# usnistgov/optbayesexpt

Hardware: AMD Instinct MI355X
Metric: model-evals/sec (settings x particles) per opt_setting+update cycle, fp64 (higher is better)
Workload: dtype f64; 1 GPU; c3: Lorentzian 3-param, 65 536 settings x 1 048 576 particles; n_settings=65536, n_particles=1048576, settings_per_rank=65536

## Files before the change

### optbayesexpt_amd/csrc/obe_sweep_bins.h

```cpp
#pragma once
#include "obe_sweep_common.h"

namespace obe {

struct BinPlan {
    double origin;
    int nbins;
    unsigned poison;
};
constexpr int kBinMinmaxBlocks = 256;
constexpr int kBinMaxUnits = 2048;
constexpr int kBinChunk = 1024;
constexpr int kBinFoldGroups = 16;
constexpr int kBinScanPer = kBinMaxUnits / kBlock;
constexpr double kBinEvalSlots = 8.0 * LorentzBins::kOrder + 16.0;
constexpr double kBinDrawSlots = 4.0 * LorentzBins::kOrder + 8.0;
constexpr double kBinFixedSlots = 80.0 * 3.9e7;

struct BinUnits {
    int nunits;
    int64_t per;
};
static BinUnits plan_bin_units(int64_t nd) {
    BinUnits u;
    u.per = (nd + kBinMaxUnits - 1) / kBinMaxUnits;
    u.per = std::max<int64_t>(kWave, (u.per + kWave - 1) / kWave * kWave);
    u.nunits = static_cast<int>((nd + u.per - 1) / u.per);
    return u;
}
struct BinEvalShape {
    int waves, groups;
};
constexpr BinEvalShape kBinEvalShapes[] = {{8, 1}, {6, 2}, {3, 4}};
constexpr int kBinEvalWavesPerCU = 12, kChipCUs = 256;
static int plan_bin_eval_waves(int64_t ns) {
    const int64_t groups = (ns + kWave - 1) / kWave;
    for (const BinEvalShape& f : kBinEvalShapes)
        if (groups <= (int64_t)kChipCUs * f.groups * (kBinEvalWavesPerCU / (f.groups * f.waves))) return f.waves;
    return 1;
}
static int64_t bin_max_items(int64_t nd) { return (nd + kBinChunk - 1) / kBinChunk + LorentzBins::kMaxBins; }
struct BinLayout {
    static constexpr int64_t kPlan = 0, kRan = 3, kStarts = 4;
    static constexpr int64_t kMinmax = kStarts + 132;
    static constexpr int64_t kTotals = kMinmax + 3 * kBinMinmaxBlocks;
    static constexpr int64_t kCounts = kTotals + LorentzBins::kMaxBins / 2;
    static constexpr int64_t kCoef = kCounts + (int64_t)LorentzBins::kMaxBins * kBinMaxUnits / 2;
    static constexpr int64_t kPart = kCoef + (int64_t)LorentzBins::kMaxBins * LorentzBins::kRow;
    static int64_t sorted(int64_t nd) { return kPart + bin_max_items(nd) * LorentzBins::kRow; }
    static int64_t doubles(int64_t nd) { return sorted(nd) + 4 * nd; }
};
static_assert(BinLayout::kPart % 2 == 0 && LorentzBins::kRow % 2 == 0, "the sorted records are 16-byte aligned");

struct BinKeep {
    BinPlan plan;
    unsigned mark;
    int nd;
    unsigned long long dbits;
    unsigned mismatch;
    unsigned records;
    unsigned pad[6];
};
static_assert(sizeof(BinKeep) == 64, "the head of the keep buffer is 16 ints");
constexpr unsigned kBinKeepMark = 0x6b455042u;
struct BinKeepLayout {
    static constexpr int64_t kStarts = sizeof(BinKeep) / sizeof(int);
    static constexpr int64_t kDest = (kStarts + 2 * (LorentzBins::kMaxBins + 2) + 3) & ~(int64_t)3;
    static int64_t bytes(int64_t nd) { return ((kDest + nd) * (int64_t)sizeof(int) + 15) & ~(int64_t)15; }
    static constexpr int64_t kRecord = 3;
    static int64_t records_at(int64_t nd) { return bytes(nd); }
    static int64_t sw_at(int64_t nd) { return records_at(nd) + ((kRecord * 8 * nd + 15) & ~(int64_t)15); }
    static int64_t records_bytes(int64_t nd) { return sw_at(nd) + ((8 * nd + 15) & ~(int64_t)15); }
};

#ifndef OBE_PLUGIN_MODEL_HEADER
struct BinSweepPtrs {
    BinPlan* plan;
    unsigned* ran;
    int* binstart;
    int* itemstart;
    BinKeep* keep;
    int* dest;
    int* code;
    int reuse;
    int keep_nd;
    unsigned long long keep_dbits;
    unsigned call;
    double* minmax;
    int* totals;
    int* counts;
    double* coef;
    double* part;
    double* sorted;
};

struct BinRecords {
    double* rec;
    double* sw;
    const double* bbar;
};

__device__ __forceinline__ bool bin_keep_refused(const BinSweepPtrs& q) {
    if (!q.reuse) return false;
    const BinKeep* k = q.keep;
    return !(k->mark == kBinKeepMark && k->nd == q.keep_nd && k->dbits == q.keep_dbits);
}

__device__ __forceinline__ double bin_x0(const SweepArgs& a, int64_t p) {
    double w;
    const int64_t src = draw_source(a, p, w);
    return a.particles[src];
}
__device__ __forceinline__ double bin_tau0(const SweepArgs& a, int64_t p) { return bin_x0(a, p) / a.m.consts[0]; }

__device__ __forceinline__ void bin_pk(double tau0, double amp, double b, double bbar, double sw, double (&pk)[4]) {
    pk[0] = tau0;
    pk[1] = sw * amp;
    pk[2] = sw * (b - bbar);
    pk[3] = sw;
}
__device__ __forceinline__ void bin_particle(const SweepArgs& a, int64_t p, double (&part)[3], double& sw) {
    using M = Lorentz<1>;
    static_assert(packed_width<M>() == 4 && M::NPK == 3, "the sorted records are 32 bytes");
    double w;
    const int64_t src = draw_source(a, p, w);
    sw = sqrt(w);
    part[0] = a.particles[src] / a.m.consts[0];
    part[1] = a.particles[src + a.ld_p];
    part[2] = a.particles[src + 2 * a.ld_p];
}
__device__ __forceinline__ void bin_record(const SweepArgs& a, int64_t p, double2& ra, double2& rb) {
    double part[3], sw, pk[4];
    bin_particle(a, p, part, sw);
    bin_pk(part[0], part[1], part[2], a.moments[4], sw, pk);
    ra = double2{pk[0], pk[1]};
    rb = double2{pk[2], pk[3]};
}

__device__ __forceinline__ void bin_store_particle(const SweepArgs& a, int64_t p, int pos, const BinRecords& r) {
    double part[3], sw;
    bin_particle(a, p, part, sw);
    double* __restrict__ out = r.rec + BinKeepLayout::kRecord * (int64_t)pos;
    out[0] = part[0];
    out[1] = part[1];
    out[2] = part[2];
    r.sw[pos] = sw;
}

constexpr int kBinRankBits = 24;
static_assert((((int64_t)1 << 30) + kBinMaxUnits - 1) / kBinMaxUnits <= ((int64_t)1 << kBinRankBits)
                  && LorentzBins::kMaxBins <= (1 << (31 - kBinRankBits)),
              "a unit of a cloud of 2^30 draws (BinForm::selected) has at most 2^19 draws: rank and bin share an int");
__device__ __forceinline__ int bin_code(int bin, int rank) { return (bin << kBinRankBits) | rank; }
constexpr int kBinIndexBits = 7;
constexpr int kBinGroupAhead = 8;
static_assert(LorentzBins::kMaxBins == 1 << kBinIndexBits, "a bin index is matched bit by bit (bin_group_kernel<false>)");

__global__ __launch_bounds__(kBlock) void bin_minmax_kernel(SweepArgs a, BinSweepPtrs q) {
    constexpr int NW = kBlock / kWave;
    __shared__ double slo[NW], shi[NW];
    __shared__ int sbad[NW];
    if (sweep_aborted(a.abort)) return;
    if (q.keep && blockIdx.x == 0 && threadIdx.x == 0) {
        q.keep->mark = 0u;
        q.keep->records = 0u;
    }
    double* __restrict__ minmax = q.minmax;
    double lo = INFINITY, hi = -INFINITY;
    int bad = 0;
    for (int64_t p = (int64_t)blockIdx.x * kBlock + threadIdx.x; p < a.nd; p += (int64_t)gridDim.x * kBlock) {
        const double t = bin_tau0(a, p);
        bad |= !(fabs(t) <= kDblMax);
        lo = fmin(lo, t);
        hi = fmax(hi, t);
    }
#pragma unroll
    for (int o = kWave / 2; o > 0; o >>= 1) {
        lo = fmin(lo, __shfl_down(lo, o, kWave));
        hi = fmax(hi, __shfl_down(hi, o, kWave));
        bad |= __shfl_down(bad, o, kWave);
    }
    if ((threadIdx.x & (kWave - 1)) == 0) {
        slo[threadIdx.x / kWave] = lo;
        shi[threadIdx.x / kWave] = hi;
        sbad[threadIdx.x / kWave] = bad;
    }
    __syncthreads();
    if (threadIdx.x != 0) return;
    for (int g = 1; g < NW; ++g) {
        lo = fmin(lo, slo[g]);
        hi = fmax(hi, shi[g]);
        bad |= sbad[g];
    }
    minmax[blockIdx.x] = lo;
    minmax[kBinMinmaxBlocks + blockIdx.x] = hi;
    minmax[2 * kBinMinmaxBlocks + blockIdx.x] = bad ? 1.0 : 0.0;
}

__device__ __forceinline__ BinPlan bin_plan_of(const SweepArgs& a, const double* __restrict__ minmax, int nblocks) {
    const int lane = threadIdx.x & (kWave - 1);
    double lo = INFINITY, hi = -INFINITY;
    int bad = 0;
#pragma unroll
    for (int g = 0; g < kBinMinmaxBlocks / kWave; ++g) {
        const int b = g * kWave + lane;
        const bool have = b < nblocks;
        lo = fmin(lo, have ? minmax[b] : INFINITY);
        hi = fmax(hi, have ? minmax[kBinMinmaxBlocks + b] : -INFINITY);
        bad |= have ? minmax[2 * kBinMinmaxBlocks + b] != 0.0 : 0;
    }
#pragma unroll
    for (int o = kWave / 2; o > 0; o >>= 1) {
        lo = fmin(lo, __shfl_xor(lo, o, kWave));
        hi = fmax(hi, __shfl_xor(hi, o, kWave));
        bad |= __shfl_xor(bad, o, kWave);
    }
    const double d = a.m.consts[0];
    const double n = floor((hi - lo) * (1.0 / LorentzBins::kWidth)) + 1.0;
    const bool ok = !bad && d > 0.0 && d <= kDblMax && fabs(lo) <= kDblMax && fabs(hi) <= kDblMax
                    && n <= (double)LorentzBins::kMaxBins;
    return BinPlan{lo, ok ? static_cast<int>(n) : 0, ok ? 0u : 1u};
}

__device__ __forceinline__ int wave_exclusive(int v, int& total) {
    const int lane = threadIdx.x & (kWave - 1);
    int inc = v;
#pragma unroll
    for (int o = 1; o < kWave; o <<= 1) {
        const int up = __shfl_up(inc, o, kWave);
        inc += lane >= o ? up : 0;
    }
    total = __shfl(inc, kWave - 1, kWave);
    return inc - v;
}

template <bool SCATTER, bool RECORDS = false>
__global__ __launch_bounds__(kBlock) void bin_group_kernel(SweepArgs a, int64_t per, int nunits, int mm_blocks,
                                                           BinSweepPtrs q, BinRecords r) {
    using LB = LorentzBins;
    static_assert(SCATTER || !RECORDS, "the counting pass stores no record");
    if (sweep_aborted(a.abort)) return;
    const int lane = threadIdx.x & (kWave - 1);
    const int unit = blockIdx.x * (kBlock / kWave) + threadIdx.x / kWave;
    BinPlan plan;
    if constexpr (SCATTER) {
        plan = *q.plan;
        if (q.keep && blockIdx.x == 0 && threadIdx.x == 0) {
            q.keep->nd = static_cast<int>(a.nd);
            q.keep->dbits = q.keep_dbits;
            q.keep->mismatch = 0u;
            q.keep->mark = kBinKeepMark;
            if constexpr (RECORDS) q.keep->records = kBinKeepMark;
        }
    } else {
        plan = bin_plan_of(a, q.minmax, mm_blocks);
        if (blockIdx.x == 0 && threadIdx.x == 0) *q.plan = plan;
    }
    const int nbins = __builtin_amdgcn_readfirstlane(plan.nbins);
    if (nbins == 0) return;
    int c0 = 0, c1 = 0;
    if constexpr (SCATTER) {
        const int t0 = q.totals[lane], t1 = q.totals[lane + kWave];
        int sum0, sum1, isum0, isum1;
        const int e0 = wave_exclusive(t0, sum0), e1 = sum0 + wave_exclusive(t1, sum1);
        const int i0 = wave_exclusive((t0 + kBinChunk - 1) / kBinChunk, isum0);
        const int i1 = isum0 + wave_exclusive((t1 + kBinChunk - 1) / kBinChunk, isum1);
        if (unit == 0) {
            q.binstart[lane] = e0;
            q.binstart[lane + kWave] = e1;
            q.itemstart[lane] = i0;
            q.itemstart[lane + kWave] = i1;
            if (lane == 0) {
                q.binstart[LB::kMaxBins] = sum0 + sum1;
                q.itemstart[LB::kMaxBins] = isum0 + isum1;
            }
        }
        if (unit >= nunits) return;
        c0 = e0 + q.counts[lane * kBinMaxUnits + unit];
        c1 = e1 + q.counts[(lane + kWave) * kBinMaxUnits + unit];
    }
    if (unit >= nunits) return;
    const int64_t begin = (int64_t)unit * per;
    const int64_t end = begin + per < a.nd ? begin + per : a.nd;
    if constexpr (SCATTER) {
        for (int64_t i0 = begin; i0 < end; i0 += kWave) {
            const int64_t i = i0 + lane;
            const bool live = i < end;
            const int code = live ? q.code[i] : 0;
            const int bin = code >> kBinRankBits;
            const int first0 = __shfl(c0, bin & (kWave - 1), kWave), first1 = __shfl(c1, bin & (kWave - 1), kWave);
            const int pos = (bin < kWave ? first0 : first1) + (code & ((1 << kBinRankBits) - 1));
            if (live && pos >= 0 && pos < a.nd) {
                if constexpr (RECORDS) {
                    bin_store_particle(a, i, pos, r);
                } else {
                    double2 ra, rb;
                    bin_record(a, i, ra, rb);
                    double2* __restrict__ out = reinterpret_cast<double2*>(q.sorted) + 2 * (int64_t)pos;
                    out[0] = ra;
                    out[1] = rb;
                }
            }
            if (q.dest && live) q.dest[i] = pos;
        }
    } else {
        __shared__ int tally[kBlock / kWave][LB::kMaxBins];
        int* count = tally[threadIdx.x / kWave];
        count[lane] = 0;
        count[lane + kWave] = 0;
        __builtin_amdgcn_fence(__ATOMIC_SEQ_CST, "wavefront");
        const double d = a.m.consts[0];
        const unsigned long long below = (1ull << lane) - 1ull;
        auto trip = [&](int64_t i0, double x0) {
            const int64_t i = i0 + lane;
            const bool live = i < end;
            const int bin = live ? LB::bin_of(plan.origin, x0 / d, nbins) : -1;
            unsigned long long same = __ballot(live);
#pragma unroll
            for (int k = 0; k < kBinIndexBits; ++k) {
                const bool bit = (bin >> k) & 1;
                const unsigned long long have = __ballot(bit);
                same &= bit ? have : ~have;
            }
            if (!live) same = 0ull;
            const int sofar = live ? count[bin] : 0;
            if (live && (same & below) == 0ull) count[bin] = sofar + __popcll(same);
            __builtin_amdgcn_fence(__ATOMIC_SEQ_CST, "wavefront");
            if (live) q.code[i] = bin_code(bin, sofar + __popcll(same & below));
        };
        for (int64_t i0 = begin; i0 < end; i0 += kBinGroupAhead * kWave) {
            double x0[kBinGroupAhead];
#pragma unroll
            for (int k = 0; k < kBinGroupAhead; ++k) {
                const int64_t i = i0 + k * kWave + lane;
                x0[k] = bin_x0(a, i < end ? i : end - 1);
            }
#pragma unroll
            for (int k = 0; k < kBinGroupAhead; ++k)
                if (i0 + k * kWave < end) trip(i0 + k * kWave, x0[k]);
        }
        q.counts[lane * kBinMaxUnits + unit] = count[lane];
        q.counts[(lane + kWave) * kBinMaxUnits + unit] = count[lane + kWave];
    }
}

template <bool RECORDS>
__device__ __forceinline__ void bin_scatter_pack_draw(const SweepArgs& a, const BinSweepPtrs& q, const BinRecords& r,
                                                      double origin, int nbins, int64_t p) {
    using LB = LorentzBins;
    double2 ra, rb;
    bin_record(a, p, ra, rb);
    const int pos = q.dest[p];
    const double t = (ra.x - origin) * (1.0 / LB::kWidth);
    bool ok = t >= 0.0 && t < (double)nbins && pos >= 0 && pos < a.nd;
    if (ok) {
        const int b = LB::bin_of(origin, ra.x, nbins);
        ok = q.binstart[b] <= pos && pos < q.binstart[b + 1];
    }
    if (ok) {
        if constexpr (RECORDS) {
            bin_store_particle(a, p, pos, r);
        } else {
            double2* __restrict__ out = reinterpret_cast<double2*>(q.sorted) + 2 * (int64_t)pos;
            out[0] = ra;
            out[1] = rb;
        }
    } else {
        q.keep->mismatch = q.call;
    }
}
__global__ __launch_bounds__(kBlock) void bin_scatter_pack_kernel(SweepArgs a, BinSweepPtrs q) {
    using LB = LorentzBins;
    if (sweep_aborted(a.abort)) return;
    if (bin_keep_refused(q)) return;
    const int nbins = __builtin_amdgcn_readfirstlane(q.plan->nbins);
    if (nbins <= 0 || nbins > LB::kMaxBins) return;
    const double origin = q.plan->origin;
    for (int64_t p = (int64_t)blockIdx.x * kBlock + threadIdx.x; p < a.nd; p += (int64_t)gridDim.x * kBlock)
        bin_scatter_pack_draw<false>(a, q, BinRecords{}, origin, nbins, p);
}

__global__ __launch_bounds__(kBlock) void bin_refresh_kernel(SweepArgs a, BinSweepPtrs q, BinRecords r, int64_t per) {
    using LB = LorentzBins;
    if (sweep_aborted(a.abort)) return;
    if (bin_keep_refused(q)) return;
    const int nbins = __builtin_amdgcn_readfirstlane(q.plan->nbins);
    if (nbins <= 0 || nbins > LB::kMaxBins) return;
    const int64_t begin = (int64_t)blockIdx.x * per;
    const int64_t end = begin + per < a.nd ? begin + per : a.nd;
    if (q.keep->records == kBinKeepMark) {
        const double* __restrict__ w = a.weights;
        const int* __restrict__ dest = q.dest;
        for (int64_t p = begin + threadIdx.x; p < end; p += kBlock) {
            const int pos = dest[p];
            if (pos >= 0 && pos < a.nd) r.sw[pos] = sqrt(w[p]);
        }
    } else {
        const double origin = q.plan->origin;
        for (int64_t p = begin + threadIdx.x; p < end; p += kBlock) bin_scatter_pack_draw<true>(a, q, r, origin, nbins, p);
    }
}

__global__ __launch_bounds__(kBlock) void bin_scan_kernel(int nunits, BinSweepPtrs q, const unsigned* abort) {
    __shared__ int wsum[kBlock / kWave];
    if (sweep_aborted(abort)) return;
    const int nbins = __builtin_amdgcn_readfirstlane(q.plan->nbins);
    const int bin = blockIdx.x;
    if (nbins == 0) return;
    if (bin >= nbins) {
        if (threadIdx.x == 0) q.totals[bin] = 0;
        return;
    }
    int* __restrict__ row = q.counts + bin * kBinMaxUnits;
    int v[kBinScanPer], mine = 0;
#pragma unroll
    for (int u = 0; u < kBinScanPer; ++u) {
        const int k = threadIdx.x * kBinScanPer + u;
        v[u] = k < nunits ? row[k] : 0;
        mine += v[u];
    }
    int wtotal;
    int before = wave_exclusive(mine, wtotal);
    if ((threadIdx.x & (kWave - 1)) == 0) wsum[threadIdx.x / kWave] = wtotal;
    __syncthreads();
    int total = 0;
#pragma unroll
    for (int g = 0; g < kBlock / kWave; ++g) {
        if (g < (int)threadIdx.x / kWave) before += wsum[g];
        total += wsum[g];
    }
#pragma unroll
    for (int u = 0; u < kBinScanPer; ++u) {
        const int k = threadIdx.x * kBinScanPer + u;
        if (k < nunits) row[k] = before;
        before += v[u];
    }
    if (threadIdx.x == 0) q.totals[bin] = total;
}

template <int N, int DIST>
__device__ __forceinline__ void halving_reduce(const double (&v)[N], int lane, double (&out)[2]) {
    constexpr int H = (N + 1) / 2;
    const bool upper = (lane & DIST) != 0;
    double k[H];
#pragma unroll
    for (int i = 0; i < H; ++i) {
        const double lo = v[i], hi = H + i < N ? v[H + i] : 0.0;
        const double mine = upper ? hi : lo, send = upper ? lo : hi;
        k[i] = mine + __shfl_xor(send, DIST, kWave);
    }
    if constexpr (DIST > 1) {
        halving_reduce<H, DIST / 2>(k, lane, out);
    } else {
        static_assert(H == 2, "64 lanes x 2 values: at most 128 sums");
        out[0] = k[0];
        out[1] = k[1];
    }
}
template <int N>
__device__ __forceinline__ int halving_index(int lane, int e) {
    int n[7];
    n[0] = N;
#pragma unroll
    for (int l = 0; l < 6; ++l) n[l + 1] = (n[l] + 1) / 2;
    int j = e;
    bool real = true;
#pragma unroll
    for (int l = 5; l >= 0; --l) {
        j += ((lane >> (5 - l)) & 1) * n[l + 1];
        real = real && j < n[l];
    }
    return real ? j : -1;
}

template <bool RECORDS>
__global__ __launch_bounds__(kWave) void bin_moments_kernel(BinSweepPtrs q, const unsigned* abort, BinRecords r) {
    using LB = LorentzBins;
    if (sweep_aborted(abort)) return;
    if (bin_keep_refused(q)) return;
    const int nbins = __builtin_amdgcn_readfirstlane(q.plan->nbins);
    if (nbins == 0) return;
    const int lane = threadIdx.x, item = blockIdx.x;
    if (item >= q.itemstart[LB::kMaxBins]) return;
    const int s0 = q.itemstart[lane], s1 = q.itemstart[lane + kWave];
    const int bin = __popcll(__ballot(lane < nbins && s0 <= item)) + __popcll(__ballot(lane + kWave < nbins && s1 <= item)) - 1;
    const int first = q.binstart[bin] + (item - q.itemstart[bin]) * kBinChunk;
    const int last = q.binstart[bin + 1];
    const int end = first + kBinChunk < last ? first + kBinChunk : last;
    const double tb = LB::centre(q.plan->origin, bin);
    LB::Sums z;
    z.clear();
    if constexpr (!RECORDS) {
        const double2* __restrict__ rec = reinterpret_cast<const double2*>(q.sorted);
        int i = first + lane;
        double2 ra = double2{0.0, 0.0}, rb = ra;
        if (i < end) {
            ra = rec[2 * (int64_t)i];
            rb = rec[2 * (int64_t)i + 1];
        }
        while (i < end) {
            const int in = i + kWave;
            double2 na = ra, nb = rb;
            if (in < end) {
                na = rec[2 * (int64_t)in];
                nb = rec[2 * (int64_t)in + 1];
            }
            const double pk[4] = {ra.x, ra.y, rb.x, rb.y};
            LB::add_draw(tb, pk, z);
            ra = na;
            rb = nb;
            i = in;
        }
    } else {
        const double bbar = *r.bbar;
        const double* __restrict__ rec = r.rec;
        const double* __restrict__ rsw = r.sw;
        constexpr int64_t R = BinKeepLayout::kRecord;
        int i = first + lane;
        double tau0 = 0.0, amp = 0.0, b = 0.0, sw = 0.0;
        if (i < end) {
            tau0 = rec[R * i];
            amp = rec[R * i + 1];
            b = rec[R * i + 2];
            sw = rsw[i];
        }
        while (i < end) {
            const int in = i + kWave;
            double ntau0 = tau0, namp = amp, nb = b, nsw = sw;
            if (in < end) {
                ntau0 = rec[R * in];
                namp = rec[R * in + 1];
                nb = rec[R * in + 2];
                nsw = rsw[in];
            }
            double pk[4];
            bin_pk(tau0, amp, b, bbar, sw, pk);
            LB::add_draw(tb, pk, z);
            tau0 = ntau0;
            amp = namp;
            b = nb;
            sw = nsw;
            i = in;
        }
    }
    double v[LB::kCoefs], kept[2];
#pragma unroll
    for (int k = 0; k < LB::kOrder; ++k) {
        v[k] = z.M1[k];
        v[LB::kOrder + k] = z.M2[k];
        v[2 * LB::kOrder + k] = z.M3[k];
    }
    v[3 * LB::kOrder] = z.c1;
    v[3 * LB::kOrder + 1] = z.c2;
    halving_reduce<LB::kCoefs, kWave / 2>(v, lane, kept);
    double* __restrict__ out = q.part + (int64_t)item * LB::kRow;
#pragma unroll
    for (int e = 0; e < 2; ++e) {
        const int j = halving_index<LB::kCoefs>(lane, e);
        if (j < 0) continue;
        const bool m3 = j >= 2 * LB::kOrder && j < 3 * LB::kOrder;
        out[j] = kept[e] * (m3 ? (double)(j - 2 * LB::kOrder + 1) : 1.0);
    }
}

__global__ __launch_bounds__(kBinFoldGroups * kWave) void bin_fold_kernel(BinSweepPtrs q, const unsigned* abort) {
    using LB = LorentzBins;
    __shared__ double acc[kBinFoldGroups][kWave];
    if (sweep_aborted(abort)) return;
    if (bin_keep_refused(q)) return;
    const int nbins = __builtin_amdgcn_readfirstlane(q.plan->nbins);
    const int bin = blockIdx.x >> 1, co = (blockIdx.x & 1) * kWave + (threadIdx.x & (kWave - 1));
    if (bin >= nbins) return;
    const int first = __builtin_amdgcn_readfirstlane(q.itemstart[bin]);
    const int n = __builtin_amdgcn_readfirstlane(q.itemstart[bin + 1]) - first;
    if (n == 0) return;
    const bool live = co < LB::kCoefs;
    const double t = fold_in_order<kBinFoldGroups>(q.part + (int64_t)first * LB::kRow + co, n, LB::kRow, live, acc);
    if (threadIdx.x < kWave && live) q.coef[(int64_t)bin * LB::kRow + co] = t;
}

constexpr int kBinTile = 16;
template <int G, int W>
__global__ __launch_bounds__(G * W * kWave, W == 1 ? 1 : 3)
void bin_eval_kernel(SweepArgs a, BinSweepPtrs q, unsigned seq, BinFinish f) {
    using LB = LorentzBins;
    constexpr int kThreads = G * W * kWave;
    static_assert(W > 1 || kThreads == kBlock, "W = 1 is the workgroup of four groups");
    static_assert((G * W) % 4 == 0, "whole wavefronts for every SIMD of the CU (plan_bin_eval_waves)");
    static_assert(LB::kMaxBins <= 2 * kWave && kWave % kBinTile == 0, "two ballots name the occupied bins");
    const int lane = threadIdx.x & (kWave - 1);
    const int wave = __builtin_amdgcn_readfirstlane((int)threadIdx.x / kWave);
    const int grp = wave % G, wid = wave / G;
    double* term = nullptr;
    if constexpr (W == 1) {
        if (sweep_aborted(a.abort)) return;
    } else {
        __shared__ double terms[G * 2 * kBinTile * kWave];
        __shared__ int stop;
        term = terms + grp * (2 * kBinTile * kWave);
        if (threadIdx.x == 0) stop = sweep_aborted(a.abort);
        __syncthreads();
        if (stop) return;
    }
    const int64_t s = ((int64_t)blockIdx.x * G + grp) * kWave + lane;
    const bool refused = bin_keep_refused(q) || (q.reuse && q.keep->mismatch == q.call);
    const int nbins = refused ? 0 : __builtin_amdgcn_readfirstlane(q.plan->nbins);
    double S1 = __builtin_nan(""), S2 = __builtin_nan("");
    if (nbins > 0) {
        double tau;
        Lorentz<1>::prep_setting(a.settings + (s < a.ns ? s : a.ns - 1), a.m, &tau);
        const double origin = q.plan->origin;
        const double* __restrict__ coef = q.coef;
        const int* __restrict__ start = q.binstart;
        const bool here0 = lane < nbins && start[lane + 1] != start[lane];
        const bool here1 = kWave + lane < nbins && start[kWave + lane + 1] != start[kWave + lane];
        const uint64_t occ0 = __ballot(here0), occ1 = __ballot(here1);
        uint64_t own0 = occ0, own1 = occ1;
        double c1col[2] = {0.0, 0.0}, c2col[2] = {0.0, 0.0};
        if constexpr (W > 1) {
            uint64_t mine = 0;
            for (int t = wid; t < kBinTile; t += W) mine |= (uint64_t)1 << t;
            mine |= mine << 16;
            mine |= mine << 32;
            own0 &= mine;
            own1 &= mine;
            if (wid == 0) {
                if (here0) {
                    c1col[0] = coef[lane * LB::kRow + 3 * LB::kOrder];
                    c2col[0] = coef[lane * LB::kRow + 3 * LB::kOrder + 1];
                }
                if (here1) {
                    c1col[1] = coef[(kWave + lane) * LB::kRow + 3 * LB::kOrder];
                    c2col[1] = coef[(kWave + lane) * LB::kRow + 3 * LB::kOrder + 1];
                }
            }
        }
        auto next_bin = [&]() {
            int b = -1;
            if (own0) {
                b = __builtin_ctzll(own0);
                own0 &= own0 - 1;
            } else if (own1) {
                b = kWave + __builtin_ctzll(own1);
                own1 &= own1 - 1;
            }
            return b;
        };
        double a1 = 0.0, a2 = 0.0, C1 = 0.0, C2 = 0.0;
        int tile = 0;
        auto close_tile = [&]() {
            __syncthreads();
            if (wid == 0) {
                const int half = tile * kBinTile / kWave;
                const uint64_t occ = half ? occ1 : occ0;
                for (int t = 0; t < kBinTile; ++t) {
                    const int l = (tile * kBinTile + t) & (kWave - 1);
                    if (!((occ >> l) & 1)) continue;
                    a1 += term[t * kWave + lane];
                    a2 += term[(kBinTile + t) * kWave + lane];
                    C1 += readlane_f64(half ? c1col[1] : c1col[0], l);
                    C2 += readlane_f64(half ? c2col[1] : c2col[0], l);
                }
            }
            __syncthreads();
            ++tile;
        };
        auto evaluate = [&](const LB::LaneRow& row, int b) {
            double t1, t2;
            if constexpr (W == 1) {
                LB::evaluate(row, LB::centre(origin, b) - tau, t1, t2);
                a1 += t1;
                a2 += t2;
                LB::add_constants(row, C1, C2);
            } else {
                while (tile < b / kBinTile) close_tile();
                LB::evaluate(row, LB::centre(origin, b) - tau, t1, t2);
                term[(b % kBinTile) * kWave + lane] = t1;
                term[(kBinTile + b % kBinTile) * kWave + lane] = t2;
            }
        };
        LB::LaneRow row0, row1;
        int b0 = next_bin();
        if (b0 >= 0) {
            LB::load_row(coef + b0 * LB::kRow, lane, row0);
            for (;;) {
                const int b1 = next_bin();
                LB::load_row(coef + (b1 >= 0 ? b1 : b0) * LB::kRow, lane, row1);
                evaluate(row0, b0);
                if (b1 < 0) break;
                b0 = next_bin();
                LB::load_row(coef + (b0 >= 0 ? b0 : b1) * LB::kRow, lane, row0);
                evaluate(row1, b1);
                if (b0 < 0) break;
            }
        }
        if constexpr (W > 1)
            while (tile < (nbins + kBinTile - 1) / kBinTile) close_tile();
        S1 = a1 + C1;
        S2 = a2 + C2;
    }
    if (blockIdx.x == 0 && threadIdx.x == 0) *q.ran = seq;
    if (W > 1 && wid != 0) return;
    if (!f.yvar) {
        if (s >= a.ns) return;
        a.part1[s] = S1;
        a.part2[s] = S2;
        a.cs_out[s] = 0.0;
        return;
    }
    const int64_t group = (int64_t)blockIdx.x * G + grp;
    if (group * kWave >= a.ns) return;
    double kappa = 0.0;
    Best best{-INFINITY, INT64_MAX};
    if (s < a.ns) {
        const double var = variance_of_moments(0.0 + S1, 0.0 + S2, f.full_mode ? a.moments[0] : 1.0, 0.0, kappa);
        f.yvar[s] = var;
        const double u = utility_of(&var, 1, 1, s, f.ua);
        f.utility[s] = u;
        best = Best{u, s};
    }
    wave_best(best, kappa);
    if (lane == 0) {
        f.bv[group] = best.v;
        f.bi[group] = best.i;
        f.bk[group] = kappa;
    }
}

struct BinForm {
    bool on = false;
    BinSweepPtrs q{};
    BinRecords r{};

    static bool selected(const obe_model& m, int flags, int64_t ns, const int64_t* d_draw_idx, int64_t n_draws,
                         int64_t nd) {
        return (flags & OBE_SWEEP_BINS) && nd <= ((int64_t)1 << 30) && expansion_applies(m, flags, ns, d_draw_idx, n_draws);
    }
    void carve(double* base, double* packed, int64_t nd, const obe_model& m, int flags, const int64_t* d_draw_idx,
               void* d_keep, int64_t keep_bytes) {
        using BL = BinLayout;
        q.plan = reinterpret_cast<BinPlan*>(base + BL::kPlan);
        q.ran = reinterpret_cast<unsigned*>(base + BL::kRan);
        q.binstart = reinterpret_cast<int*>(base + BL::kStarts);
        q.itemstart = q.binstart + LorentzBins::kMaxBins + 2;
        q.minmax = base + BL::kMinmax;
        q.totals = reinterpret_cast<int*>(base + BL::kTotals);
        q.counts = reinterpret_cast<int*>(base + BL::kCounts);
        q.coef = base + BL::kCoef;
        q.part = base + BL::kPart;
        q.sorted = base + BL::sorted(nd);
        q.code = reinterpret_cast<int*>(packed);
        if (d_keep && !d_draw_idx && keep_bytes >= BinKeepLayout::bytes(nd)) {
            static std::atomic<unsigned> calls{0};
            int* ints = static_cast<int*>(d_keep);
            q.keep = static_cast<BinKeep*>(d_keep);
            q.plan = &q.keep->plan;
            q.binstart = ints + BinKeepLayout::kStarts;
            q.itemstart = q.binstart + LorentzBins::kMaxBins + 2;
            q.dest = ints + BinKeepLayout::kDest;
            q.code = q.dest;
            q.reuse = (flags & OBE_SWEEP_BINS_KEPT) != 0;
            q.keep_nd = static_cast<int>(nd);
            memcpy(&q.keep_dbits, &m.consts[0], sizeof q.keep_dbits);
            q.call = ++calls;
            if (q.call == 0u) q.call = ++calls;
            if (keep_bytes >= BinKeepLayout::records_bytes(nd)) {
                char* bytes = static_cast<char*>(d_keep);
                r.rec = reinterpret_cast<double*>(bytes + BinKeepLayout::records_at(nd));
                r.sw = reinterpret_cast<double*>(bytes + BinKeepLayout::sw_at(nd));
            }
        }
    }
    int before(const SweepArgs& a, hipStream_t st) const {
        if (!q.reuse) return 0;
        if (r.rec) {
            const int64_t per = plan_bin_units(a.nd).per * (kBlock / kWave);
            bin_refresh_kernel<<<(unsigned)((a.nd + per - 1) / per), kBlock, 0, st>>>(a, q, r, per);
            OBE_CHECK_LAUNCH("bin_refresh_kernel");
            return 0;
        }
        bin_scatter_pack_kernel<<<stream_blocks(a.nd, kBlock), kBlock, 0, st>>>(a, q);
        OBE_CHECK_LAUNCH("bin_scatter_pack_kernel");
        return 0;
    }
    int sweep(SweepPlan& p, const SweepArgs& a, unsigned seq, const BinFinish& f, hipStream_t st) const {
        using LB = LorentzBins;
        if (!q.reuse) {
            const BinUnits units = plan_bin_units(a.nd);
            const int mm_blocks = static_cast<int>(std::min<int64_t>(kBinMinmaxBlocks, (a.nd + kBlock - 1) / kBlock));
            bin_minmax_kernel<<<mm_blocks, kBlock, 0, st>>>(a, q);
            OBE_CHECK_LAUNCH("bin_minmax_kernel");
            const unsigned group_blocks = (unsigned)((units.nunits + kBlock / kWave - 1) / (kBlock / kWave));
            bin_group_kernel<false><<<group_blocks, kBlock, 0, st>>>(a, units.per, units.nunits, mm_blocks, q, r);
            OBE_CHECK_LAUNCH("bin_group_kernel<count>");
            bin_scan_kernel<<<LB::kMaxBins, kBlock, 0, st>>>(units.nunits, q, a.abort);
            OBE_CHECK_LAUNCH("bin_scan_kernel");
            if (r.rec)
                bin_group_kernel<true, true><<<group_blocks, kBlock, 0, st>>>(a, units.per, units.nunits, mm_blocks, q, r);
            else
                bin_group_kernel<true><<<group_blocks, kBlock, 0, st>>>(a, units.per, units.nunits, mm_blocks, q, r);
            OBE_CHECK_LAUNCH("bin_group_kernel<scatter>");
        }
        if (r.rec) {
            BinRecords rr = r;
            rr.bbar = a.moments + 4;
            bin_moments_kernel<true><<<(unsigned)bin_max_items(a.nd), kWave, 0, st>>>(q, a.abort, rr);
        } else {
            bin_moments_kernel<false><<<(unsigned)bin_max_items(a.nd), kWave, 0, st>>>(q, a.abort, r);
        }
        OBE_CHECK_LAUNCH("bin_moments_kernel");
        bin_fold_kernel<<<2 * LB::kMaxBins, kBinFoldGroups * kWave, 0, st>>>(q, a.abort);
        OBE_CHECK_LAUNCH("bin_fold_kernel");
        p.nchunks = 1;
        const unsigned groups = (unsigned)((a.ns + kWave - 1) / kWave);
        switch (plan_bin_eval_waves(a.ns)) {
            case 8: bin_eval_kernel<1, 8><<<groups, 8 * kWave, 0, st>>>(a, q, seq, f); break;
            case 6: bin_eval_kernel<2, 6><<<(groups + 1) / 2, 12 * kWave, 0, st>>>(a, q, seq, f); break;
            case 3: bin_eval_kernel<4, 3><<<(groups + 3) / 4, 12 * kWave, 0, st>>>(a, q, seq, f); break;
            default: bin_eval_kernel<4, 1><<<(groups + 3) / 4, kBlock, 0, st>>>(a, q, seq, f);
        }
        OBE_CHECK_LAUNCH("bin_eval_kernel");
        return 0;
    }
};
#endif

}
```

Baseline: 624400 billion model-evals/s.

## Gather weights by source index in moments kernel instead of refreshing sqrt-weight array

The kept sorted records now store each draw's source index instead of a precomputed sqrt(weight). The moments kernel gathers the current weight through that index and takes the square root inline, with the next index prefetched one step ahead. This removes the per-cycle refresh kernel that rewrote the sqrt-weight array through a scatter. A host-side hint table records which keep buffers hold valid records, so the validating scatter kernel only launches when that is unknown. In exchange, the weight reads become random gathers, and a host mutex is added.

```diff
diff --git a/optbayesexpt_amd/csrc/obe_sweep_bins.h b/optbayesexpt_amd/csrc/obe_sweep_bins.h
--- a/optbayesexpt_amd/csrc/obe_sweep_bins.h
+++ b/optbayesexpt_amd/csrc/obe_sweep_bins.h
@@ -1,4 +1,6 @@
 #pragma once
+#include <mutex>
+
 #include "obe_sweep_common.h"
 
 namespace obe {
@@ -69,8 +71,8 @@
     static int64_t bytes(int64_t nd) { return ((kDest + nd) * (int64_t)sizeof(int) + 15) & ~(int64_t)15; }
     static constexpr int64_t kRecord = 3;
     static int64_t records_at(int64_t nd) { return bytes(nd); }
-    static int64_t sw_at(int64_t nd) { return records_at(nd) + ((kRecord * 8 * nd + 15) & ~(int64_t)15); }
-    static int64_t records_bytes(int64_t nd) { return sw_at(nd) + ((8 * nd + 15) & ~(int64_t)15); }
+    static int64_t src_at(int64_t nd) { return records_at(nd) + ((kRecord * 8 * nd + 15) & ~(int64_t)15); }
+    static int64_t records_bytes(int64_t nd) { return src_at(nd) + ((8 * nd + 15) & ~(int64_t)15); }
 };
 
 #ifndef OBE_PLUGIN_MODEL_HEADER
@@ -96,14 +98,19 @@
 
 struct BinRecords {
     double* rec;
-    double* sw;
+    int* src;
+    const double* w;
     const double* bbar;
+    int checked;
 };
 
 __device__ __forceinline__ bool bin_keep_refused(const BinSweepPtrs& q) {
     if (!q.reuse) return false;
     const BinKeep* k = q.keep;
     return !(k->mark == kBinKeepMark && k->nd == q.keep_nd && k->dbits == q.keep_dbits);
+}
+__device__ __forceinline__ bool bin_records_refused(const BinSweepPtrs& q, const BinRecords& r) {
+    return q.reuse && !r.checked && q.keep->records != kBinKeepMark;
 }
 
 __device__ __forceinline__ double bin_x0(const SweepArgs& a, int64_t p) {
@@ -144,7 +151,7 @@
     out[0] = part[0];
     out[1] = part[1];
     out[2] = part[2];
-    r.sw[pos] = sw;
+    r.src[pos] = static_cast<int>(p);
 }
 
 constexpr int kBinRankBits = 24;
@@ -380,25 +387,16 @@
         bin_scatter_pack_draw<false>(a, q, BinRecords{}, origin, nbins, p);
 }
 
-__global__ __launch_bounds__(kBlock) void bin_refresh_kernel(SweepArgs a, BinSweepPtrs q, BinRecords r, int64_t per) {
+__global__ __launch_bounds__(kBlock) void bin_check_records_kernel(SweepArgs a, BinSweepPtrs q, BinRecords r) {
     using LB = LorentzBins;
     if (sweep_aborted(a.abort)) return;
     if (bin_keep_refused(q)) return;
+    if (q.keep->records == kBinKeepMark) return;
     const int nbins = __builtin_amdgcn_readfirstlane(q.plan->nbins);
     if (nbins <= 0 || nbins > LB::kMaxBins) return;
-    const int64_t begin = (int64_t)blockIdx.x * per;
-    const int64_t end = begin + per < a.nd ? begin + per : a.nd;
-    if (q.keep->records == kBinKeepMark) {
-        const double* __restrict__ w = a.weights;
-        const int* __restrict__ dest = q.dest;
-        for (int64_t p = begin + threadIdx.x; p < end; p += kBlock) {
-            const int pos = dest[p];
-            if (pos >= 0 && pos < a.nd) r.sw[pos] = sqrt(w[p]);
-        }
-    } else {
-        const double origin = q.plan->origin;
-        for (int64_t p = begin + threadIdx.x; p < end; p += kBlock) bin_scatter_pack_draw<true>(a, q, r, origin, nbins, p);
-    }
+    const double origin = q.plan->origin;
+    for (int64_t p = (int64_t)blockIdx.x * kBlock + threadIdx.x; p < a.nd; p += (int64_t)gridDim.x * kBlock)
+        bin_scatter_pack_draw<true>(a, q, r, origin, nbins, p);
 }
 
 __global__ __launch_bounds__(kBlock) void bin_scan_kernel(int nunits, BinSweepPtrs q, const unsigned* abort) {
@@ -478,6 +476,12 @@
     using LB = LorentzBins;
     if (sweep_aborted(abort)) return;
     if (bin_keep_refused(q)) return;
+    if constexpr (RECORDS) {
+        if (bin_records_refused(q, r)) {
+            if (blockIdx.x == 0 && threadIdx.x == 0) q.keep->mismatch = q.call;
+            return;
+        }
+    }
     const int nbins = __builtin_amdgcn_readfirstlane(q.plan->nbins);
     if (nbins == 0) return;
     const int lane = threadIdx.x, item = blockIdx.x;
@@ -514,34 +518,46 @@
     } else {
         const double bbar = *r.bbar;
         const double* __restrict__ rec = r.rec;
-        const double* __restrict__ rsw = r.sw;
+        const int* __restrict__ src = r.src;
+        const double* __restrict__ w = r.w;
+        const unsigned nd = (unsigned)q.keep_nd;
         constexpr int64_t R = BinKeepLayout::kRecord;
         int i = first + lane;
-        double tau0 = 0.0, amp = 0.0, b = 0.0, sw = 0.0;
+        double tau0 = 0.0, amp = 0.0, b = 0.0, wt = 0.0;
+        int snext = 0;
+        bool astray = false;
         if (i < end) {
             tau0 = rec[R * i];
             amp = rec[R * i + 1];
             b = rec[R * i + 2];
-            sw = rsw[i];
+            const int s = src[i];
+            if ((unsigned)s < nd) wt = w[s];
+            else astray = true;
+            if (i + kWave < end) snext = src[i + kWave];
         }
         while (i < end) {
             const int in = i + kWave;
-            double ntau0 = tau0, namp = amp, nb = b, nsw = sw;
+            double ntau0 = tau0, namp = amp, nb = b, nwt = wt;
+            int safter = snext;
             if (in < end) {
                 ntau0 = rec[R * in];
                 namp = rec[R * in + 1];
                 nb = rec[R * in + 2];
-                nsw = rsw[in];
+                if ((unsigned)snext < nd) nwt = w[snext];
+                else astray = true;
+                if (in + kWave < end) safter = src[in + kWave];
             }
             double pk[4];
-            bin_pk(tau0, amp, b, bbar, sw, pk);
+            bin_pk(tau0, amp, b, bbar, sqrt(wt), pk);
             LB::add_draw(tb, pk, z);
             tau0 = ntau0;
             amp = namp;
             b = nb;
-            sw = nsw;
+            wt = nwt;
+            snext = safter;
             i = in;
         }
+        if (astray) q.keep->mismatch = q.call;
     }
     double v[LB::kCoefs], kept[2];
 #pragma unroll
@@ -727,6 +743,44 @@
     }
 }
 
+struct RecordsHint {
+    static constexpr int kSlots = 16;
+    struct Slot {
+        const void* keep = nullptr;
+        int nd = 0;
+        unsigned long long dbits = 0;
+    };
+    struct Table {
+        std::mutex lock;
+        Slot slot[kSlots];
+        unsigned next = 0;
+    };
+    static Table& table() {
+        static Table t;
+        return t;
+    }
+    static void rebuilt(const void* keep, bool records, int nd, unsigned long long dbits) {
+        Table& t = table();
+        std::lock_guard<std::mutex> guard(t.lock);
+        Slot* at = nullptr;
+        for (Slot& s : t.slot)
+            if (s.keep == keep) at = &s;
+        if (!records) {
+            if (at) *at = Slot{};
+            return;
+        }
+        if (!at) at = &t.slot[t.next++ % kSlots];
+        *at = Slot{keep, nd, dbits};
+    }
+    static bool fits(const void* keep, int nd, unsigned long long dbits) {
+        Table& t = table();
+        std::lock_guard<std::mutex> guard(t.lock);
+        for (const Slot& s : t.slot)
+            if (s.keep == keep) return s.nd == nd && s.dbits == dbits;
+        return false;
+    }
+};
+
 struct BinForm {
     bool on = false;
     BinSweepPtrs q{};
@@ -767,16 +821,17 @@
             if (keep_bytes >= BinKeepLayout::records_bytes(nd)) {
                 char* bytes = static_cast<char*>(d_keep);
                 r.rec = reinterpret_cast<double*>(bytes + BinKeepLayout::records_at(nd));
-                r.sw = reinterpret_cast<double*>(bytes + BinKeepLayout::sw_at(nd));
+                r.src = reinterpret_cast<int*>(bytes + BinKeepLayout::src_at(nd));
+                r.checked = q.reuse && !RecordsHint::fits(d_keep, q.keep_nd, q.keep_dbits);
             }
         }
     }
     int before(const SweepArgs& a, hipStream_t st) const {
         if (!q.reuse) return 0;
         if (r.rec) {
-            const int64_t per = plan_bin_units(a.nd).per * (kBlock / kWave);
-            bin_refresh_kernel<<<(unsigned)((a.nd + per - 1) / per), kBlock, 0, st>>>(a, q, r, per);
-            OBE_CHECK_LAUNCH("bin_refresh_kernel");
+            if (!r.checked) return 0;
+            bin_check_records_kernel<<<stream_blocks(a.nd, kBlock), kBlock, 0, st>>>(a, q, r);
+            OBE_CHECK_LAUNCH("bin_check_records_kernel");
             return 0;
         }
         bin_scatter_pack_kernel<<<stream_blocks(a.nd, kBlock), kBlock, 0, st>>>(a, q);
@@ -786,6 +841,7 @@
     int sweep(SweepPlan& p, const SweepArgs& a, unsigned seq, const BinFinish& f, hipStream_t st) const {
         using LB = LorentzBins;
         if (!q.reuse) {
+            if (q.keep) RecordsHint::rebuilt(q.keep, r.rec != nullptr, q.keep_nd, q.keep_dbits);
             const BinUnits units = plan_bin_units(a.nd);
             const int mm_blocks = static_cast<int>(std::min<int64_t>(kBinMinmaxBlocks, (a.nd + kBlock - 1) / kBlock));
             bin_minmax_kernel<<<mm_blocks, kBlock, 0, st>>>(a, q);
@@ -803,6 +859,7 @@
         }
         if (r.rec) {
             BinRecords rr = r;
+            rr.w = a.weights;
             rr.bbar = a.moments + 4;
             bin_moments_kernel<true><<<(unsigned)bin_max_items(a.nd), kWave, 0, st>>>(q, a.abort, rr);
         } else {
```

New measurement: 666600 billion model-evals/s (median of 5 runs). +6.8%, better.
